# facebookresearch/multipathnet

Hardware: NVIDIA H100
Metric: proposals/sec (higher is better)
Workload: dtype fp32 (wgmma split emulation, fp32 accumulate: 3 bf16 products per MAC, 2 fp16 products in fc6/fc7)

## Files before the change

multipathnet_b200/csrc/gemm_tc.cu:

```cuda
#include "conv_gemm.cuh"
#include "wgmma.cuh"
#include "fp8_e4m3.cuh"
#include <algorithm>
#include <stdlib.h>
#include <string.h>

namespace {

constexpr int BM = 128;
constexpr int BK = 64;
constexpr int TC_THREADS = 384;
constexpr int CONS_THREADS = 256;
constexpr int A_TILE_BYTES = BM * BK * 2;
constexpr int SMEM_BUDGET = 196608;

__host__ __device__ constexpr int a_planes(OperandScheme ops) { return (ops == OperandScheme::BF16X1 || ops == OperandScheme::FP8X1) ? 1 : 2; }
__host__ __device__ constexpr int b_planes(OperandScheme ops) { return ops == OperandScheme::BF16X3 ? 2 : 1; }
__host__ __device__ constexpr int elem_bytes(OperandScheme ops) { return ops == OperandScheme::FP8X1 ? 1 : 2; }
__host__ __device__ constexpr int row_bytes(int BN, OperandScheme ops) { return (ops == OperandScheme::FP8X1 || BN == 256) ? 64 : 128; }
__host__ __device__ constexpr int stage_k(int BN, OperandScheme ops) { return row_bytes(BN, ops) / elem_bytes(ops); }
__host__ __device__ constexpr int kb_steps(int BN, OperandScheme ops) { return BK / stage_k(BN, ops); }
__host__ __device__ constexpr int a_tile_bytes(int BN, OperandScheme ops) { return BM * row_bytes(BN, ops); }
__host__ __device__ constexpr int stage_bytes(int BN, OperandScheme ops = OperandScheme::BF16X3) {
  return (a_planes(ops) * BM + b_planes(ops) * BN) * row_bytes(BN, ops);
}
__host__ __device__ constexpr int max_stages(int BN, OperandScheme ops) { return row_bytes(BN, ops) == 64 ? 8 : 4; }
__host__ __device__ constexpr int num_stages(int BN, OperandScheme ops = OperandScheme::BF16X3) {
  return (SMEM_BUDGET / stage_bytes(BN, ops)) > max_stages(BN, ops) ? max_stages(BN, ops) : (SMEM_BUDGET / stage_bytes(BN, ops));
}
__host__ __device__ constexpr int tc_smem_bytes(int BN, OperandScheme ops) {
  return num_stages(BN, ops) * stage_bytes(BN, ops) + 1024  + 256 ;
}
__host__ __device__ constexpr int stg_ld(int BN) { return BN + 4; }

struct TcParams {
  int N, Ho, Wo, Cout;
  int kh, kw, stride, pad;
  int cblocks;
  int tn, th, tw;
  int tiles_img, tiles_h, tiles_w, tiles_n;
  const float *bias;
  const __nv_bfloat16 *res_hi, *res_lo; long long res_ld;
  __nv_bfloat16 *out_hi, *out_lo; long long out_ld;
  float *out_f32; long long out_f32_ld;
  __nv_bfloat16 *pool_hi, *pool_lo; long long pool_ld; int Hp, Wp;
  int relu;
  int splitk, kb_per_split;
  long long split_stride;
  unsigned long long *tl_min, *tl_max;
  float acc_scale;
  int out_fmt;
  unsigned *ovf;
  const int *a_exp, *b_exp; long long sample_pix;
};

__device__ __forceinline__ unsigned long long gtimer() {
  unsigned long long t; asm volatile("mov.u64 %0, %%globaltimer;" : "=l"(t)); return t;
}
__device__ __forceinline__ void tl_min_stamp(const unsigned long long *base_, int i) {
  if (base_) atomicMin(const_cast<unsigned long long *>(base_) + i, gtimer());
}
__device__ __forceinline__ void tl_max_stamp(const unsigned long long *base_, int i) {
  if (base_) atomicMax(const_cast<unsigned long long *>(base_) + i, gtimer());
}
__device__ __forceinline__ uint32_t smem_u32(const void *p) { return (uint32_t)__cvta_generic_to_shared(p); }
__device__ __forceinline__ void mbar_init(uint32_t bar, uint32_t count) {
  asm volatile("mbarrier.init.shared::cta.b64 [%0], %1;" ::"r"(bar), "r"(count) : "memory");
}
__device__ __forceinline__ void mbar_expect_tx(uint32_t bar, uint32_t bytes) {
  asm volatile("mbarrier.arrive.expect_tx.shared::cta.b64 _, [%0], %1;" ::"r"(bar), "r"(bytes) : "memory");
}
__device__ __forceinline__ void mbar_arrive(uint32_t bar) {
  asm volatile("mbarrier.arrive.shared::cta.b64 _, [%0];" ::"r"(bar) : "memory");
}
__device__ __forceinline__ void mbar_wait(uint32_t bar, uint32_t parity) {
  uint32_t done;
  uint32_t spins = 0;
  do {
    asm volatile(
        "{\n\t.reg .pred p;\n\t"
        "mbarrier.try_wait.parity.shared::cta.b64 p, [%1], %2;\n\t"
        "selp.u32 %0, 1, 0, p;\n\t}"
        : "=r"(done) : "r"(bar), "r"(parity) : "memory");
    if (!done && ++spins == (1u << 26)) __trap();
  } while (!done);
}
__device__ __forceinline__ void tma_load_4d(uint32_t dst, const CUtensorMap *tm, uint32_t bar, int c0, int c1,
                                            int c2, int c3) {
  asm volatile(
      "cp.async.bulk.tensor.4d.shared::cluster.global.mbarrier::complete_tx::bytes [%0], [%1, {%3, %4, %5, %6}], [%2];"
      ::"r"(dst), "l"(reinterpret_cast<uint64_t>(tm)), "r"(bar), "r"(c0), "r"(c1), "r"(c2), "r"(c3) : "memory");
}
__device__ __forceinline__ void tma_load_2d(uint32_t dst, const CUtensorMap *tm, uint32_t bar, int c0, int c1) {
  asm volatile(
      "cp.async.bulk.tensor.2d.shared::cluster.global.mbarrier::complete_tx::bytes [%0], [%1, {%3, %4}], [%2];"
      ::"r"(dst), "l"(reinterpret_cast<uint64_t>(tm)), "r"(bar), "r"(c0), "r"(c1) : "memory");
}
__device__ __forceinline__ void prefetch_tmap(const CUtensorMap *tm) {
  asm volatile("prefetch.tensormap [%0];" ::"l"(reinterpret_cast<uint64_t>(tm)) : "memory");
}
__device__ __forceinline__ void consumers_sync() { asm volatile("bar.sync 1, 256;" ::: "memory"); }

__device__ __forceinline__ uint64_t make_smem_desc(uint32_t saddr) {
  uint64_t d = 0;
  d |= (uint64_t)((saddr & 0x3FFFFu) >> 4);
  d |= (uint64_t)1 << 16;
  d |= (uint64_t)(1024 >> 4) << 32;
  d |= (uint64_t)1 << 62;
  return d;
}

__device__ __forceinline__ uint64_t make_smem_desc_64b(uint32_t saddr) {
  uint64_t d = 0;
  d |= (uint64_t)((saddr & 0x3FFFFu) >> 4);
  d |= (uint64_t)1 << 16;
  d |= (uint64_t)(512 >> 4) << 32;
  d |= (uint64_t)2 << 62;
  return d;
}

template <int BN, OperandScheme OPS>
__device__ __forceinline__ void mma_kstep(float (&acc)[BN / 2], uint64_t a_hi, uint64_t a_lo, uint64_t b_hi, uint64_t b_lo, bool first) {
  constexpr bool F16 = (OPS == OperandScheme::FP16X2);
#pragma unroll
  for (int k = 0; k < stage_k(BN, OPS) / 16; ++k) {
    const uint64_t adv = (uint64_t)((k * 16 * 2) >> 4);
    const uint32_t later = (first && k == 0) ? 0u : 1u;
    if constexpr (OPS == OperandScheme::BF16X1) {
      wgmma_nk16<BN, false>(acc, a_hi + adv, b_hi + adv, later);
    } else {
      wgmma_nk16<BN, F16>(acc, a_lo + adv, b_hi + adv, later);
      if (!F16) wgmma_nk16<BN, F16>(acc, a_hi + adv, b_lo + adv, 1u);
      wgmma_nk16<BN, F16>(acc, a_hi + adv, b_hi + adv, 1u);
    }
  }
}

template <int BN>
__device__ __forceinline__ void stage_acc(float *stg, const float (&acc)[BN / 2], int g, int t) {
  const int r0 = g * 64 + (t >> 5) * 16 + ((t & 31) >> 2), c0 = 2 * (t & 3);
#pragma unroll
  for (int j = 0; j < BN / 8; ++j) {
    *reinterpret_cast<float2 *>(stg + r0 * stg_ld(BN) + 8 * j + c0) = make_float2(acc[4 * j], acc[4 * j + 1]);
    *reinterpret_cast<float2 *>(stg + (r0 + 8) * stg_ld(BN) + 8 * j + c0) = make_float2(acc[4 * j + 2], acc[4 * j + 3]);
  }
}

template <int BN, OperandScheme OPS>
__device__ __forceinline__ void epilogue_row(const TcParams &p, const float *srow, int nt, bool row_ok, long long pix,
                                             float *out_f32, int ch_first, long long ppix) {
  const bool pool = (p.pool_hi != nullptr);
  const int tile_end = min(p.Cout, nt * BN + BN);
#pragma unroll 1
  for (int ch = ch_first; ch < BN / 32; ch += 2) {
    const int col0 = nt * BN + ch * 32;
    if (col0 >= tile_end) break;
    float v[32];
#pragma unroll
    for (int j = 0; j < 8; ++j) {
      const float4 x = *reinterpret_cast<const float4 *>(srow + ch * 32 + 4 * j);
      v[4 * j] = x.x; v[4 * j + 1] = x.y; v[4 * j + 2] = x.z; v[4 * j + 3] = x.w;
    }
    if (OPS == OperandScheme::FP16X2) {
#pragma unroll
      for (int e = 0; e < 32; ++e) v[e] *= p.acc_scale;
    }
    if (OPS == OperandScheme::FP8X1) {
      const int ea = row_ok ? __ldg(p.a_exp + pix / p.sample_pix) : 0;
#pragma unroll
      for (int e = 0; e < 32; ++e) v[e] *= mpn_fp8::pow2(-(ea + __ldg(p.b_exp + col0 + e)));
    }
    if (!(row_ok || pool)) continue;
#pragma unroll
    for (int g = 0; g < 4; ++g) {
      const int c = col0 + g * 8;
      if (c >= tile_end) break;
      float f[8];
#pragma unroll
      for (int e = 0; e < 8; ++e) f[e] = v[g * 8 + e];
      const bool full8 = (c + 8 <= tile_end);
      if (p.bias) {
        if (full8) {
          const float4 b0 = __ldg(reinterpret_cast<const float4 *>(p.bias + c));
          const float4 b1 = __ldg(reinterpret_cast<const float4 *>(p.bias + c + 4));
          f[0] += b0.x; f[1] += b0.y; f[2] += b0.z; f[3] += b0.w;
          f[4] += b1.x; f[5] += b1.y; f[6] += b1.z; f[7] += b1.w;
        } else {
          for (int e = 0; e < 8 && c + e < p.Cout; ++e) f[e] += __ldg(p.bias + c + e);
        }
      }
      if (p.res_hi && full8 && row_ok) {
        const uint4 rh = *reinterpret_cast<const uint4 *>(p.res_hi + pix * p.res_ld + c);
        const uint4 rl = *reinterpret_cast<const uint4 *>(p.res_lo + pix * p.res_ld + c);
        const uint32_t hh[4] = {rh.x, rh.y, rh.z, rh.w}, ll[4] = {rl.x, rl.y, rl.z, rl.w};
#pragma unroll
        for (int t = 0; t < 4; ++t) {
          float2 x = bf16x2_to_float2(hh[t]), y = bf16x2_to_float2(ll[t]);
          f[2 * t] += x.x + y.x; f[2 * t + 1] += x.y + y.y;
        }
      }
      if (p.relu) {
#pragma unroll
        for (int e = 0; e < 8; ++e) f[e] = fmaxf(f[e], 0.f);
      }
      if (p.out_hi && full8 && row_ok) {
        uint32_t oh[4], ol[4];
#pragma unroll
        for (int t = 0; t < 4; ++t) split_x2(p.out_fmt, f[2 * t], f[2 * t + 1], oh[t], ol[t], p.ovf);
        *reinterpret_cast<uint4 *>(p.out_hi + pix * p.out_ld + c) = make_uint4(oh[0], oh[1], oh[2], oh[3]);
        *reinterpret_cast<uint4 *>(p.out_lo + pix * p.out_ld + c) = make_uint4(ol[0], ol[1], ol[2], ol[3]);
      }
      if (pool) {
#pragma unroll
        for (int e = 0; e < 8; ++e) {
          float x = row_ok ? f[e] : -INFINITY;
          x = fmaxf(x, __shfl_xor_sync(0xffffffffu, x, 1));
          x = fmaxf(x, __shfl_xor_sync(0xffffffffu, x, 8));
          f[e] = x;
        }
        if (ppix >= 0 && full8) {
          uint32_t oh[4], ol[4];
#pragma unroll
          for (int t = 0; t < 4; ++t) split_x2(p.out_fmt, f[2 * t], f[2 * t + 1], oh[t], ol[t], p.ovf);
          *reinterpret_cast<uint4 *>(p.pool_hi + ppix * p.pool_ld + c) = make_uint4(oh[0], oh[1], oh[2], oh[3]);
          *reinterpret_cast<uint4 *>(p.pool_lo + ppix * p.pool_ld + c) = make_uint4(ol[0], ol[1], ol[2], ol[3]);
        }
      }
      if (out_f32 && row_ok) {
        float *o = out_f32 + pix * p.out_f32_ld + c;
        if (full8 && ((reinterpret_cast<uintptr_t>(o) & 15) == 0)) {
          reinterpret_cast<float4 *>(o)[0] = make_float4(f[0], f[1], f[2], f[3]);
          reinterpret_cast<float4 *>(o)[1] = make_float4(f[4], f[5], f[6], f[7]);
        } else {
          for (int e = 0; e < 8 && c + e < p.Cout; ++e) o[e] = f[e];
        }
      }
    }
  }
}

template <int BN, OperandScheme OPS = OperandScheme::BF16X3>
__global__ void __launch_bounds__(TC_THREADS, 1)
conv_gemm_tc_kernel(const __grid_constant__ CUtensorMap tmA_hi, const __grid_constant__ CUtensorMap tmA_lo,
                    const __grid_constant__ CUtensorMap tmB_hi, const __grid_constant__ CUtensorMap tmB_lo,
                    const TcParams p) {
  constexpr int S = num_stages(BN, OPS);
  constexpr int STAGE = stage_bytes(BN, OPS);
  constexpr int A_TILE = a_tile_bytes(BN, OPS);
  constexpr int B_TILE_BYTES = BN * row_bytes(BN, OPS);
  constexpr int B_OFF = a_planes(OPS) * A_TILE;
  constexpr int KSTEPS = kb_steps(BN, OPS);
  static_assert(BM * stg_ld(BN) * 4 <= S * STAGE, "staging tile must fit in the ring");
  static_assert(S >= 2 && 2 * S * 8 <= 256, "ring depth: at least two stages, barriers in their 256 bytes");
  extern __shared__ uint8_t smem_raw[];
  uint8_t *smem = reinterpret_cast<uint8_t *>((reinterpret_cast<uintptr_t>(smem_raw) + 1023) & ~(uintptr_t)1023);
  uint64_t *bars = reinterpret_cast<uint64_t *>(smem + (size_t)S * STAGE);
  const uint32_t smem_base = smem_u32(smem);
  const uint32_t bar_base = smem_u32(bars);
  auto full_bar = [&](int s) { return bar_base + 8u * s; };
  auto empty_bar = [&](int s) { return bar_base + 8u * (S + s); };

  const int tid = threadIdx.x, lane = tid & 31;
  const int unit = (int)blockIdx.x;
  const int tile = unit / p.splitk, split = unit - tile * p.splitk;
  const int nt = tile % p.tiles_n, mt = tile / p.tiles_n;
  const int twi = mt % p.tiles_w, thi = (mt / p.tiles_w) % p.tiles_h, tni = mt / (p.tiles_w * p.tiles_h);
  const int num_kb = p.kh * p.kw * p.cblocks;
  const int kb0 = split * p.kb_per_split, kb1 = min(num_kb, kb0 + p.kb_per_split);

  if (tid == 0) {
    tl_min_stamp(p.tl_min, 0);
    if (a_planes(OPS) == 1) { prefetch_tmap(&tmA_hi); prefetch_tmap(&tmB_hi); }
    else { prefetch_tmap(&tmA_hi); prefetch_tmap(&tmA_lo); prefetch_tmap(&tmB_hi); prefetch_tmap(&tmB_lo); }
    for (int s = 0; s < S; ++s) { mbar_init(full_bar(s), 1); mbar_init(empty_bar(s), CONS_THREADS / 32); }
    asm volatile("fence.mbarrier_init.release.cluster;" ::: "memory");
  }
  __syncthreads();
  asm volatile("griddepcontrol.wait;" ::: "memory");
  asm volatile("griddepcontrol.launch_dependents;" ::: "memory");
  if (tid == 0) tl_min_stamp(p.tl_min, 1);

  if (tid < 128) {
    if (tid == 0) {
      const int w_in0 = twi * p.tw * p.stride - p.pad, h_in0 = thi * p.th * p.stride - p.pad, n0 = tni * p.tn;
      const int b_row0 = nt * BN;
      for (int kb = kb0, it = 0; kb < kb1; ++kb) {
        const int tap = kb / p.cblocks, cb = kb - tap * p.cblocks;
        const int khi = tap / p.kw, kwi = tap - khi * p.kw;
#pragma unroll
        for (int h = 0; h < KSTEPS; ++h, ++it) {
          const int s = it % S; const uint32_t ph = (uint32_t)(it / S) & 1u;
          const int ka = cb * BK + h * stage_k(BN, OPS), kk = kb * BK + h * stage_k(BN, OPS);
          mbar_wait(empty_bar(s), ph ^ 1u);
          const uint32_t sa = smem_base + (uint32_t)s * STAGE;
          mbar_expect_tx(full_bar(s), (uint32_t)STAGE);
          tma_load_4d(sa, &tmA_hi, full_bar(s), ka, w_in0 + kwi, h_in0 + khi, n0);
          if (a_planes(OPS) == 2) tma_load_4d(sa + A_TILE, &tmA_lo, full_bar(s), ka, w_in0 + kwi, h_in0 + khi, n0);
          tma_load_2d(sa + B_OFF, &tmB_hi, full_bar(s), kk, b_row0);
          if (b_planes(OPS) == 2) tma_load_2d(sa + B_OFF + B_TILE_BYTES, &tmB_lo, full_bar(s), kk, b_row0);
        }
      }
    }
    return;
  }

  const int e = tid - 128;
  const int g = e >> 7, t = e & 127;
  float acc[BN / 2];
#pragma unroll
  for (int i = 0; i < BN / 2; ++i) acc[i] = 0.f;
  if constexpr (OPS == OperandScheme::FP8X1) {
    float part[BN / 2];
#pragma unroll
    for (int i = 0; i < BN / 2; ++i) part[i] = 0.f;
    for (int kb = kb0, it = 0; kb < kb1; ++kb, ++it) {
      const int s = it % S; const uint32_t ph = (uint32_t)(it / S) & 1u;
      mbar_wait(full_bar(s), ph);
      if (it == 0 && e == 0) tl_min_stamp(p.tl_min, 2);
      const uint32_t sa = smem_base + (uint32_t)s * STAGE;
      const uint64_t a8 = make_smem_desc_64b(sa + (uint32_t)g * (A_TILE / 2));
      const uint64_t b8 = make_smem_desc_64b(sa + B_OFF);
#pragma unroll
      for (int k = 0; k < BK / 32; ++k) {
        wgmma_fence_acc(part);
        wgmma_fence();
        wgmma_e4m3_nk32<BN>(part, a8 + (uint64_t)(2 * k), b8 + (uint64_t)(2 * k), 0u);
        wgmma_commit();
        wgmma_wait<0>();
        wgmma_fence_acc(part);
#pragma unroll
        for (int i = 0; i < BN / 2; ++i) acc[i] += part[i];
      }
      if (lane == 0) mbar_arrive(empty_bar(s));
    }
  } else {
  const int steps = (kb1 - kb0) * KSTEPS;
  for (int it = 0; it < steps; ++it) {
    const int s = it % S; const uint32_t ph = (uint32_t)(it / S) & 1u;
    mbar_wait(full_bar(s), ph);
    if (it == 0 && e == 0) tl_min_stamp(p.tl_min, 2);
    const uint32_t sa = smem_base + (uint32_t)s * STAGE;
    auto desc = [](uint32_t a) { return row_bytes(BN, OPS) == 64 ? make_smem_desc_64b(a) : make_smem_desc(a); };
    const uint64_t a_hi = desc(sa + (uint32_t)g * (A_TILE / 2));
    const uint64_t a_lo = desc(sa + A_TILE + (uint32_t)g * (A_TILE / 2));
    const uint64_t b_hi = desc(sa + B_OFF);
    const uint64_t b_lo = desc(sa + B_OFF + B_TILE_BYTES);
    wgmma_fence_acc(acc);
    wgmma_fence();
    mma_kstep<BN, OPS>(acc, a_hi, a_lo, b_hi, b_lo, it == 0);
    wgmma_commit();
    wgmma_wait<1>();
    wgmma_fence_acc(acc);
    if (it > 0 && lane == 0) mbar_arrive(empty_bar((it - 1) % S));
  }
  wgmma_wait<0>();
  wgmma_fence_acc(acc);
  }
  if (e == 0) tl_max_stamp(p.tl_max, 0);
  consumers_sync();
  float *stg = reinterpret_cast<float *>(smem);
  stage_acc<BN>(stg, acc, g, t);
  consumers_sync();

  const int row = e & 127;
  const int wl = row & (p.tw - 1), hl = (row / p.tw) & (p.th - 1), nl = row / (p.tw * p.th);
  const int wo = twi * p.tw + wl, ho = thi * p.th + hl, n = tni * p.tn + nl;
  const bool row_ok = (wo < p.Wo) && (ho < p.Ho) && (n < p.N);
  const long long pix = ((long long)n * p.Ho + ho) * p.Wo + wo;
  const long long ppix = (p.pool_hi && row_ok && !(lane & 9)) ? ((long long)n * p.Hp + (ho >> 1)) * p.Wp + (wo >> 1) : -1;
  float *const out_f32 = p.out_f32 ? p.out_f32 + (long long)split * p.split_stride : nullptr;
  epilogue_row<BN, OPS>(p, stg + row * stg_ld(BN), nt, row_ok, pix, out_f32, e >> 7, ppix);
  if (e == 0) tl_max_stamp(p.tl_max, 1);
}

constexpr int C1_THREADS = 256;
constexpr int C1_A_BYTES = 2 * A_TILE_BYTES;
constexpr int C1_B_BYTES = 2 * 64 * 128;
constexpr int C1_OUT_WARP = 16 * 128;
constexpr int C1_SMEM = 2 * C1_A_BYTES + C1_B_BYTES + (C1_THREADS / 32) * C1_OUT_WARP + 1024;

__device__ __forceinline__ void conv1_gather(const float *__restrict__ x, int pix, int pixels, int H, int W, int bhalf,
                                             float (&in)[16]) {
#pragma unroll
  for (int k = 0; k < 16; ++k) in[k] = 0.f;
  if (pix < pixels) {
    const int HW = H * W;
    const int n = pix / HW, rem = pix - n * HW;
    const int ho = rem / W, wo = rem - ho * W;
    const float *x0 = x + ((size_t)n * 3 * HW + (size_t)(ho - 1) * W + (wo - 1));
    const bool rok[3] = {ho >= 1, true, ho + 1 < H}, cok[3] = {wo >= 1, true, wo + 1 < W};
#pragma unroll
    for (int k = 0; k < 16; ++k) {
      const int kk = 16 * bhalf + k;
      if (kk < 27) {
        const int ci = kk / 9, r = (kk / 3) % 3, q = kk % 3;
        in[k] = (rok[r] && cok[q]) ? __ldg(x0 + ci * HW + r * W + q) : 0.f;
      }
    }
  }
}

__device__ __forceinline__ void conv1_store_plane(uint32_t so, const uint32_t (&v)[16], __nv_bfloat16 *out, int pix0,
                                                  int pixels, int lane) {
  const int r = lane >> 2;
  const uint32_t wr = so + (uint32_t)(r * 128 + 4 * (lane & 3));
  __syncwarp();
#pragma unroll
  for (int j = 0; j < 8; ++j) {
    const uint32_t a = wr + (uint32_t)((j ^ r) * 16);
    asm volatile("st.shared.b32 [%0], %1;" ::"r"(a), "r"(v[j]) : "memory");
    asm volatile("st.shared.b32 [%0], %1;" ::"r"(a + 8 * 128), "r"(v[8 + j]) : "memory");
  }
  __syncwarp();
  const int row0 = lane >> 3, ch = lane & 7;
  const uint32_t rd0 = so + (uint32_t)(row0 * 128 + ((ch ^ row0) * 16)), rd1 = so + (uint32_t)(row0 * 128 + ((ch ^ row0 ^ 4) * 16));
  __nv_bfloat16 *o = out + (size_t)(pix0 + row0) * 64 + ch * 8;
#pragma unroll
  for (int q = 0; q < 4; ++q) {
    uint4 d;
    asm volatile("ld.shared.v4.b32 {%0, %1, %2, %3}, [%4];" : "=r"(d.x), "=r"(d.y), "=r"(d.z), "=r"(d.w)
                 : "r"(((q & 1) ? rd1 : rd0) + (uint32_t)(q * 4 * 128)) : "memory");
    if (pix0 + row0 + 4 * q < pixels) *reinterpret_cast<uint4 *>(o + q * 4 * 64) = d;
  }
}

__global__ void __launch_bounds__(C1_THREADS, 2)
conv1_tc_kernel(const float *__restrict__ x, int N, int H, int W, const float *__restrict__ w, const float *__restrict__ bias,
                int relu, __nv_bfloat16 *__restrict__ out_hi, __nv_bfloat16 *__restrict__ out_lo) {
  extern __shared__ uint8_t smem_raw[];
  uint8_t *smem = reinterpret_cast<uint8_t *>((reinterpret_cast<uintptr_t>(smem_raw) + 1023) & ~(uintptr_t)1023);
  uint8_t *sB = smem + 2 * C1_A_BYTES;
  const int tid = threadIdx.x, lane = tid & 31, warp = tid >> 5;
  const uint32_t so = smem_u32(sB + C1_B_BYTES) + (uint32_t)(warp * C1_OUT_WARP);
  const uint32_t b_base = smem_u32(sB);
  const int g = tid >> 7;
  const int pixels = N * H * W;
  const int total_tiles = (pixels + BM - 1) / BM;
  asm volatile("griddepcontrol.wait;" ::: "memory");
  asm volatile("griddepcontrol.launch_dependents;" ::: "memory");
  const int c0 = 2 * (lane & 3);
  for (int i = tid; i < 64 * 4; i += C1_THREADS) {
    const int row = i >> 2, j = i & 3;
    uint32_t hh[4], ll[4];
#pragma unroll
    for (int q = 0; q < 4; ++q) {
      const int k0 = j * 8 + 2 * q;
      const float v0 = (k0 < 27) ? __ldg(w + row * 27 + k0) : 0.f, v1 = (k0 + 1 < 27) ? __ldg(w + row * 27 + k0 + 1) : 0.f;
      split_bf16x2(v0, v1, hh[q], ll[q]);
    }
    const uint32_t off = (uint32_t)row * 128u + (uint32_t)((j ^ (row & 7)) * 16);
    *reinterpret_cast<uint4 *>(sB + off) = make_uint4(hh[0], hh[1], hh[2], hh[3]);
    *reinterpret_cast<uint4 *>(sB + 64 * 128 + off) = make_uint4(ll[0], ll[1], ll[2], ll[3]);
  }
  const int brow = tid & 127, bhalf = tid >> 7;
  float in[16];
  conv1_gather(x, (int)blockIdx.x * BM + brow, pixels, H, W, bhalf, in);
// ... 52 lines not shown
#pragma unroll
        for (int h = 0; h < 2; ++h) {
          uint32_t hi2, lo2;
          split_bf16x2(acc[4 * j + 2 * h], acc[4 * j + 2 * h + 1], hi2, lo2);
          v[8 * h + j] = plane ? lo2 : hi2;
        }
      conv1_store_plane(so, v, plane ? out_lo : out_hi, pix0, pixels, lane);
    }
  }
}

struct ReduceParams {
  const float *ws; long long split_stride; int splitk; long long pixels; int Cout;
  const float *bias; const __nv_bfloat16 *res_hi, *res_lo; long long res_ld; int relu;
  __nv_bfloat16 *out_hi, *out_lo; long long out_ld; float *out_f32; long long out_f32_ld;
  OutScatter scatter;
};
__global__ void __launch_bounds__(256) splitk_reduce_kernel(const ReduceParams r) {
  MPN_PDL_SYNC();
  const long long idx = (long long)blockIdx.x * blockDim.x + threadIdx.x;
  if (idx >= r.pixels * r.Cout) return;
  const long long pix = idx / r.Cout; const int c = (int)(idx - pix * r.Cout);
  float acc = 0.f;
  for (int s = 0; s < r.splitk; ++s) acc += r.ws[(long long)s * r.split_stride + idx];
  if (r.bias) acc += __ldg(r.bias + c);
  if (r.res_hi) acc += join_bf16(r.res_hi[pix * r.res_ld + c], r.res_lo[pix * r.res_ld + c]);
  if (r.relu) acc = fmaxf(acc, 0.f);
  if (r.out_hi) { __nv_bfloat16 h, l; split_bf16(acc, h, l); r.out_hi[pix * r.out_ld + c] = h; r.out_lo[pix * r.out_ld + c] = l; }
  if (r.scatter.n > 0) {
#pragma unroll 1
    for (int g = 0; g < r.scatter.n; ++g)
      if (c >= r.scatter.seg[g].c0 && c < r.scatter.seg[g].c1) { r.scatter.seg[g].ptr[pix * r.scatter.seg[g].ld + (c - r.scatter.seg[g].c0)] = acc; break; }
  } else if (r.out_f32) r.out_f32[pix * r.out_f32_ld + c] = acc;
}

typedef CUresult (*PFN_encodeTiled)(CUtensorMap *, CUtensorMapDataType, cuuint32_t, void *, const cuuint64_t *,
                                    const cuuint64_t *, const cuuint32_t *, const cuuint32_t *, CUtensorMapInterleave,
                                    CUtensorMapSwizzle, CUtensorMapL2promotion, CUtensorMapFloatOOBfill);
PFN_encodeTiled get_encode_fn() {
  static PFN_encodeTiled fn = nullptr;
  if (!fn) {
    void *p = nullptr; cudaDriverEntryPointQueryResult q;
    if (cudaGetDriverEntryPoint("cuTensorMapEncodeTiled", &p, cudaEnableDefault, &q) == cudaSuccess &&
        q == cudaDriverEntryPointSuccess)
      fn = reinterpret_cast<PFN_encodeTiled>(p);
  }
  return fn;
}

int encode_map(mpn_ctx *ctx, CUtensorMap *tm, const void *base, int rank, const cuuint64_t *dims,
               const cuuint64_t *strides_bytes , const cuuint32_t *box, const cuuint32_t *estr, int BN, OperandScheme ops) {
  const bool fp8 = ops == OperandScheme::FP8X1;
  PFN_encodeTiled fn = get_encode_fn();
  if (!fn) return mpn_fail(ctx, MPN_ERR_CUDA, "cuTensorMapEncodeTiled entry point unavailable");
  CUresult r = fn(tm, fp8 ? CU_TENSOR_MAP_DATA_TYPE_UINT8 : CU_TENSOR_MAP_DATA_TYPE_BFLOAT16, (cuuint32_t)rank, const_cast<void *>(base), dims,
                  strides_bytes, box, estr, CU_TENSOR_MAP_INTERLEAVE_NONE, row_bytes(BN, ops) == 64 ? CU_TENSOR_MAP_SWIZZLE_64B : CU_TENSOR_MAP_SWIZZLE_128B,
                  CU_TENSOR_MAP_L2_PROMOTION_L2_256B, CU_TENSOR_MAP_FLOAT_OOB_FILL_NONE);
  if (r != CUDA_SUCCESS) {
    char b[256];
    snprintf(b, sizeof b, "cuTensorMapEncodeTiled failed (%d): rank %d dims %llu %llu box %u %u", (int)r, rank,
             (unsigned long long)dims[0], (unsigned long long)dims[1], box[0], box[1]);
    return mpn_fail(ctx, MPN_ERR_CUDA, b);
  }
  return MPN_OK;
}

inline bool tc_use_pdl() {
  static const int on = [] { const char *e = getenv("MPN_TC_PDL"); return (e && e[0] == '0') ? 0 : 1; }();
  return on != 0;
}

template <int BN, OperandScheme OPS = OperandScheme::BF16X3>
int launch_bn(mpn_ctx *ctx, const ConvPlan &pl, const TcParams &tp) {
  const int smem = tc_smem_bytes(BN, OPS);
  constexpr int bslot = BN == 256 ? 2 : (BN == 128 ? 1 : 0);
  constexpr int slot = OPS == OperandScheme::FP16X2 ? 3 : (OPS == OperandScheme::BF16X1 ? 5 + bslot
                                                         : (OPS == OperandScheme::FP8X1 ? 8 + bslot : bslot));
  if (!ctx->tc_attr_set[slot]) {
    MPN_CUDA(ctx, cudaFuncSetAttribute(conv_gemm_tc_kernel<BN, OPS>, cudaFuncAttributeMaxDynamicSharedMemorySize, smem));
    ctx->tc_attr_set[slot] = 1;
  }
  const long long units = (long long)pl.tiles_img * pl.tiles_h * pl.tiles_w * pl.tiles_n * pl.splitk;
  MPN_CHECK_ARG(ctx, units > 0 && units < (1ll << 31), "conv_tc: grid size out of range");
  cudaLaunchConfig_t cfg = {};
  cfg.gridDim = dim3((unsigned)units); cfg.blockDim = dim3(TC_THREADS); cfg.dynamicSmemBytes = (size_t)smem; cfg.stream = ctx->stream;
  cudaLaunchAttribute attr[1];
  int na = 0;
  if (tc_use_pdl()) {
    attr[na].id = cudaLaunchAttributeProgrammaticStreamSerialization;
    attr[na].val.programmaticStreamSerializationAllowed = 1;
    ++na;
  }
  cfg.attrs = attr; cfg.numAttrs = na;
  MPN_CUDA(ctx, cudaLaunchKernelEx(&cfg, conv_gemm_tc_kernel<BN, OPS>, pl.tmA_hi, pl.tmA_lo, pl.tmB_hi, pl.tmB_lo, tp));
  MPN_LAUNCHED(ctx);
  return MPN_OK;
}

int launch_ops(mpn_ctx *ctx, const ConvPlan &pl, const TcParams &tp) {
  if (pl.ops == OperandScheme::FP16X2) return launch_bn<256, OperandScheme::FP16X2>(ctx, pl, tp);
  if (pl.ops == OperandScheme::FP8X1)
    return pl.BN == 128 ? launch_bn<128, OperandScheme::FP8X1>(ctx, pl, tp) : launch_bn<64, OperandScheme::FP8X1>(ctx, pl, tp);
  if (pl.ops == OperandScheme::BF16X1) {
    switch (pl.BN) {
      case 256: return launch_bn<256, OperandScheme::BF16X1>(ctx, pl, tp);
      case 128: return launch_bn<128, OperandScheme::BF16X1>(ctx, pl, tp);
      default: return launch_bn<64, OperandScheme::BF16X1>(ctx, pl, tp);
    }
  }
  switch (pl.BN) {
    case 256: return launch_bn<256>(ctx, pl, tp);
    case 128: return launch_bn<128>(ctx, pl, tp);
    default: return launch_bn<64>(ctx, pl, tp);
  }
}

}

int conv1_tc_launch(mpn_ctx *ctx, const float *x_nchw, int N, int H, int W, const float *w_dev, const float *bias_dev, int relu,
                    DTensor &y) {
  MPN_CHECK_ARG(ctx, y.hi && y.lo && y.C == 64 && y.ld % 8 == 0, "conv1_tc: output must be 64-channel split planes");
  MPN_CHECK_ARG(ctx, bias_dev, "conv1_tc: bias missing");
  MPN_CHECK_ARG(ctx, y.ld == 64 && (long long)N * H * W < (1ll << 31) - 256, "conv1_tc: dense 64-channel output and < 2^31 pixels");
  if (!ctx->tc_attr_set[4]) {
    MPN_CUDA(ctx, cudaFuncSetAttribute(conv1_tc_kernel, cudaFuncAttributeMaxDynamicSharedMemorySize, C1_SMEM));
    ctx->tc_attr_set[4] = 1;
  }
  const long long tiles = ((long long)N * H * W + BM - 1) / BM;
  cudaLaunchConfig_t cfg = {};
  cfg.gridDim = dim3((unsigned)std::min<long long>(tiles, 2ll * ctx->sm_count)); cfg.blockDim = dim3(C1_THREADS);
  cfg.dynamicSmemBytes = (size_t)C1_SMEM; cfg.stream = ctx->stream;
  cudaLaunchAttribute attr[1];
  int na = 0;
  if (tc_use_pdl()) { attr[na].id = cudaLaunchAttributeProgrammaticStreamSerialization; attr[na].val.programmaticStreamSerializationAllowed = 1; ++na; }
  cfg.attrs = attr; cfg.numAttrs = na;
  MPN_CUDA(ctx, cudaLaunchKernelEx(&cfg, conv1_tc_kernel, x_nchw, N, H, W, w_dev, bias_dev, relu, y.hi, y.lo));
  MPN_LAUNCHED(ctx);
  return MPN_OK;
}

double conv_flops(const ConvProblem &p) {
  const double Ho = (double)p.y.H, Wo = (double)p.y.W;
  return 2.0 * (double)p.x.C * p.Cout * p.kh * p.kw * Ho * Wo * (double)p.y.N;
}

static int conv_tc_plan_impl(mpn_ctx *ctx, int sm_count, const ConvProblem &p, ConvPlan &pl, bool choose_only) {
  pl.valid = 0;
  MPN_CHECK_ARG(ctx, choose_only || (p.x.hi && p.x.lo && ((p.w_hi && p.w_lo) || p.w16)), "conv_tc: operands must be split-bf16 (or an fp16 weight plane)");
  MPN_CHECK_ARG(ctx, !(p.w16 && p.bf16), "conv_tc: the bf16 numerics do not take an fp16 weight plane");
  MPN_CHECK_ARG(ctx, !(p.fp8 && (p.w16 || p.bf16)), "conv_tc: the fp8 numerics take neither an fp16 weight plane nor the bf16 numerics");
  MPN_CHECK_ARG(ctx, choose_only || !p.fp8 || (p.x8 && p.x8_exp && p.w8 && p.w8_exp), "conv_tc: the fp8 numerics need e4m3 planes and exponents");
  pl.ops = p.w16 ? OperandScheme::FP16X2 : (p.fp8 ? OperandScheme::FP8X1 : (p.bf16 ? OperandScheme::BF16X1 : OperandScheme::BF16X3));
  const bool w16 = pl.ops == OperandScheme::FP16X2, fp8 = pl.ops == OperandScheme::FP8X1;
  MPN_CHECK_ARG(ctx, choose_only || (p.x.fmt == 1) == w16, "conv_tc: fp16 activation planes go with the fp16 weight plane (and only with it)");
  MPN_CHECK_ARG(ctx, p.x.C % BK == 0, "conv_tc: Cin must be a multiple of 64");
  MPN_CHECK_ARG(ctx, p.x.ld % 8 == 0, "conv_tc: input pixel stride must be a multiple of 8 elements");
  MPN_CHECK_ARG(ctx, p.stride >= 1 && p.stride <= 2, "conv_tc: stride must be 1 or 2");
  const int Ho = (int)p.y.H, Wo = (int)p.y.W, N = (int)p.y.N;
  pl.flat = (p.kh == 1 && p.kw == 1 && p.stride == 1 && p.pad == 0) ? 1 : 0;
  pl.mode = 0; pl.splitk = 1;
  cuuint64_t dims[4], strides[3]; cuuint32_t box[4], estr[4];
  int gtn = 1, gth = 1, gtw = BM;
  if (!pl.flat) {
    double best = -1.0;
    for (int tw = 1; tw <= 128; tw <<= 1)
      for (int th = 1; th * tw <= 128; th <<= 1) {
        const int tn = 128 / (tw * th);
        if (tw * p.stride > 256 || th * p.stride > 256) continue;
        const long long tiles = (long long)((Wo + tw - 1) / tw) * ((Ho + th - 1) / th) * ((N + tn - 1) / tn);
        const double util = (double)N * Ho * Wo / (double)(tiles * 128) + 1e-6 * tw;
        if (util > best) { best = util; gtn = tn; gth = th; gtw = tw; }
      }
  }
  const long long P = (long long)p.x.N * p.x.H * p.x.W;
  {
    const bool r3_ok = (p.kh == 3 && p.kw == 3 && p.stride == 1 && p.pad == 1);
    const char *env3 = getenv("MPN_TC_R3");
// ... 160 lines not shown
```

Measured before the change: 320,100.

## Make conv GEMM kernel persistent with register-direct epilogue and register reallocation

Launches at most one CTA per SM and loops over tiles, so the TMA producer can prefetch the next tile's stages while consumers run the current tile's epilogue. The epilogue no longer stages the whole fp32 accumulator tile through the ring buffer. Each warp now writes bf16 hi/lo pieces straight from registers through a small swizzled per-warp shared buffer for coalesced stores, with pooling done by warp shuffles. setmaxnreg moves registers from the producer warpgroup to the consumers. The risks are reduced parallelism when there are fewer units than SMs, more epilogue complexity, and changed bounds handling in the residual and fp32 paths.

```diff
diff --git a/multipathnet_b200/csrc/gemm_tc.cu b/multipathnet_b200/csrc/gemm_tc.cu
--- a/multipathnet_b200/csrc/gemm_tc.cu
+++ b/multipathnet_b200/csrc/gemm_tc.cu
@@ -28,10 +28,11 @@
 __host__ __device__ constexpr int num_stages(int BN, OperandScheme ops = OperandScheme::BF16X3) {
   return (SMEM_BUDGET / stage_bytes(BN, ops)) > max_stages(BN, ops) ? max_stages(BN, ops) : (SMEM_BUDGET / stage_bytes(BN, ops));
 }
+constexpr int EPI_WARP_BYTES = 16 * 128;
+constexpr int EPI_BYTES = (CONS_THREADS / 32) * EPI_WARP_BYTES;
 __host__ __device__ constexpr int tc_smem_bytes(int BN, OperandScheme ops) {
-  return num_stages(BN, ops) * stage_bytes(BN, ops) + 1024  + 256 ;
-}
-__host__ __device__ constexpr int stg_ld(int BN) { return BN + 4; }
+  return num_stages(BN, ops) * stage_bytes(BN, ops) + EPI_BYTES + 1024  + 256 ;
+}
 
 struct TcParams {
   int N, Ho, Wo, Cout;
@@ -39,6 +40,7 @@
   int cblocks;
   int tn, th, tw;
   int tiles_img, tiles_h, tiles_w, tiles_n;
+  int units;
   const float *bias;
   const __nv_bfloat16 *res_hi, *res_lo; long long res_ld;
   __nv_bfloat16 *out_hi, *out_lo; long long out_ld;
@@ -99,7 +101,6 @@
 __device__ __forceinline__ void prefetch_tmap(const CUtensorMap *tm) {
   asm volatile("prefetch.tensormap [%0];" ::"l"(reinterpret_cast<uint64_t>(tm)) : "memory");
 }
-__device__ __forceinline__ void consumers_sync() { asm volatile("bar.sync 1, 256;" ::: "memory"); }
 
 __device__ __forceinline__ uint64_t make_smem_desc(uint32_t saddr) {
   uint64_t d = 0;
@@ -136,106 +137,161 @@
   }
 }
 
-template <int BN>
-__device__ __forceinline__ void stage_acc(float *stg, const float (&acc)[BN / 2], int g, int t) {
-  const int r0 = g * 64 + (t >> 5) * 16 + ((t & 31) >> 2), c0 = 2 * (t & 3);
-#pragma unroll
-  for (int j = 0; j < BN / 8; ++j) {
-    *reinterpret_cast<float2 *>(stg + r0 * stg_ld(BN) + 8 * j + c0) = make_float2(acc[4 * j], acc[4 * j + 1]);
-    *reinterpret_cast<float2 *>(stg + (r0 + 8) * stg_ld(BN) + 8 * j + c0) = make_float2(acc[4 * j + 2], acc[4 * j + 3]);
+struct UnitPos { int nt, twi, thi, tni, split; };
+__device__ __forceinline__ UnitPos unit_pos(const TcParams &p, int unit) {
+  UnitPos u;
+  const int tile = unit / p.splitk;
+  u.split = unit - tile * p.splitk;
+  u.nt = tile % p.tiles_n;
+  const int mt = tile / p.tiles_n;
+  u.twi = mt % p.tiles_w; u.thi = (mt / p.tiles_w) % p.tiles_h; u.tni = mt / (p.tiles_w * p.tiles_h);
+  return u;
+}
+__device__ __forceinline__ long long row_pixel(const TcParams &p, const UnitPos &u, int row, bool &ok, int *whn = nullptr) {
+  const int lw = __ffs(p.tw) - 1, lh = __ffs(p.th) - 1;
+  const int wl = row & (p.tw - 1), hl = (row >> lw) & (p.th - 1), nl = row >> (lw + lh);
+  const int wo = u.twi * p.tw + wl, ho = u.thi * p.th + hl, n = u.tni * p.tn + nl;
+  ok = (wo < p.Wo) && (ho < p.Ho) && (n < p.N);
+  if (whn) { whn[0] = wo; whn[1] = ho; whn[2] = n; }
+  return ((long long)n * p.Ho + ho) * p.Wo + wo;
+}
+
+__device__ __forceinline__ void store_plane_chunk(uint32_t so, const uint32_t (&v)[16], __nv_bfloat16 *out, long long ld,
+                                                  const TcParams &p, const UnitPos &u, int rbase, int col0, int lane) {
+  const int r = lane >> 2;
+  const uint32_t wr = so + (uint32_t)(r * 128 + 4 * (lane & 3));
+  __syncwarp();
+#pragma unroll
+  for (int j = 0; j < 8; ++j) {
+    const uint32_t a = wr + (uint32_t)((j ^ r) * 16);
+    asm volatile("st.shared.b32 [%0], %1;" ::"r"(a), "r"(v[j]) : "memory");
+    asm volatile("st.shared.b32 [%0], %1;" ::"r"(a + 8 * 128), "r"(v[8 + j]) : "memory");
+  }
+  __syncwarp();
+  const int row0 = lane >> 3, ch = lane & 7;
+  const uint32_t rd0 = so + (uint32_t)(row0 * 128 + ((ch ^ row0) * 16)), rd1 = so + (uint32_t)(row0 * 128 + ((ch ^ row0 ^ 4) * 16));
+  const bool col_ok = col0 + 8 * ch < p.Cout;
+#pragma unroll
+  for (int q = 0; q < 4; ++q) {
+    uint4 d;
+    asm volatile("ld.shared.v4.b32 {%0, %1, %2, %3}, [%4];" : "=r"(d.x), "=r"(d.y), "=r"(d.z), "=r"(d.w)
+                 : "r"(((q & 1) ? rd1 : rd0) + (uint32_t)(q * 4 * 128)) : "memory");
+    bool ok;
+    const long long pix = row_pixel(p, u, rbase + 4 * q + row0, ok);
+    if (ok && col_ok) *reinterpret_cast<uint4 *>(out + pix * ld + col0 + 8 * ch) = d;
   }
 }
 
 template <int BN, OperandScheme OPS>
-__device__ __forceinline__ void epilogue_row(const TcParams &p, const float *srow, int nt, bool row_ok, long long pix,
-                                             float *out_f32, int ch_first, long long ppix) {
+__device__ __forceinline__ void tile_epilogue(const TcParams &p, const UnitPos &u, float (&acc)[BN / 2], int g, int wq,
+                                              int lane, uint32_t so) {
+  const int rbase = 64 * g + 16 * wq;
+  const int c0 = 2 * (lane & 3);
+  bool fok[2]; long long fpix[2];
+#pragma unroll
+  for (int i = 0; i < 2; ++i) fpix[i] = row_pixel(p, u, rbase + (lane >> 2) + 8 * i, fok[i]);
+  int ea[2] = {0, 0};
+  if constexpr (OPS == OperandScheme::FP8X1) {
+#pragma unroll
+    for (int i = 0; i < 2; ++i) ea[i] = fok[i] ? __ldg(p.a_exp + fpix[i] / p.sample_pix) : 0;
+  }
   const bool pool = (p.pool_hi != nullptr);
-  const int tile_end = min(p.Cout, nt * BN + BN);
+  bool pok = false; long long ppix = 0;
+  if (pool) {
+    int whn[3];
+    row_pixel(p, u, rbase + 2 * (lane >> 3), pok, whn);
+    ppix = ((long long)whn[2] * p.Hp + (whn[1] >> 1)) * p.Wp + (whn[0] >> 1);
+  }
+  float *const out_f32 = p.out_f32 ? p.out_f32 + (long long)u.split * p.split_stride : nullptr;
 #pragma unroll 1
-  for (int ch = ch_first; ch < BN / 32; ch += 2) {
-    const int col0 = nt * BN + ch * 32;
-    if (col0 >= tile_end) break;
-    float v[32];
+  for (int m = 0; m < BN / 64; ++m) {
+    const int col0 = u.nt * BN + 64 * m;
+    if (col0 >= p.Cout) break;
+    float *f = acc;
 #pragma unroll
     for (int j = 0; j < 8; ++j) {
-      const float4 x = *reinterpret_cast<const float4 *>(srow + ch * 32 + 4 * j);
-      v[4 * j] = x.x; v[4 * j + 1] = x.y; v[4 * j + 2] = x.z; v[4 * j + 3] = x.w;
-    }
-    if (OPS == OperandScheme::FP16X2) {
-#pragma unroll
-      for (int e = 0; e < 32; ++e) v[e] *= p.acc_scale;
-    }
-    if (OPS == OperandScheme::FP8X1) {
-      const int ea = row_ok ? __ldg(p.a_exp + pix / p.sample_pix) : 0;
-#pragma unroll
-      for (int e = 0; e < 32; ++e) v[e] *= mpn_fp8::pow2(-(ea + __ldg(p.b_exp + col0 + e)));
-    }
-    if (!(row_ok || pool)) continue;
-#pragma unroll
-    for (int g = 0; g < 4; ++g) {
-      const int c = col0 + g * 8;
-      if (c >= tile_end) break;
-      float f[8];
-#pragma unroll
-      for (int e = 0; e < 8; ++e) f[e] = v[g * 8 + e];
-      const bool full8 = (c + 8 <= tile_end);
-      if (p.bias) {
-        if (full8) {
-          const float4 b0 = __ldg(reinterpret_cast<const float4 *>(p.bias + c));
-          const float4 b1 = __ldg(reinterpret_cast<const float4 *>(p.bias + c + 4));
-          f[0] += b0.x; f[1] += b0.y; f[2] += b0.z; f[3] += b0.w;
-          f[4] += b1.x; f[5] += b1.y; f[6] += b1.z; f[7] += b1.w;
-        } else {
-          for (int e = 0; e < 8 && c + e < p.Cout; ++e) f[e] += __ldg(p.bias + c + e);
+      const int c = col0 + 8 * j + c0;
+      const bool full8 = col0 + 8 * j + 8 <= p.Cout;
+      float b[2] = {0.f, 0.f};
+      int eb[2] = {0, 0};
+#pragma unroll
+      for (int k = 0; k < 2; ++k) {
+        if (p.bias && c + k < p.Cout) b[k] = __ldg(p.bias + c + k);
+        if constexpr (OPS == OperandScheme::FP8X1) eb[k] = __ldg(p.b_exp + c + k);
+      }
+#pragma unroll
+      for (int i = 0; i < 2; ++i) {
+        float &f0 = f[4 * j + 2 * i], &f1 = f[4 * j + 2 * i + 1];
+        if constexpr (OPS == OperandScheme::FP16X2) { f0 *= p.acc_scale; f1 *= p.acc_scale; }
+        if constexpr (OPS == OperandScheme::FP8X1) {
+          f0 *= mpn_fp8::pow2(-(ea[i] + eb[0])); f1 *= mpn_fp8::pow2(-(ea[i] + eb[1]));
+        }
+        if (p.bias) {
+          if (c < p.Cout) f0 += b[0];
+          if (c + 1 < p.Cout) f1 += b[1];
+        }
+        if (p.res_hi && full8 && fok[i]) {
+          const float2 x = bf16x2_to_float2(*reinterpret_cast<const uint32_t *>(p.res_hi + fpix[i] * p.res_ld + c));
+          const float2 y = bf16x2_to_float2(*reinterpret_cast<const uint32_t *>(p.res_lo + fpix[i] * p.res_ld + c));
+          f0 += x.x + y.x; f1 += x.y + y.y;
+        }
+        if (p.relu) { f0 = fmaxf(f0, 0.f); f1 = fmaxf(f1, 0.f); }
+        if (out_f32 && fok[i]) {
+          float *o = out_f32 + fpix[i] * p.out_f32_ld + c;
+          if (c < p.Cout) o[0] = f0;
+          if (c + 1 < p.Cout) o[1] = f1;
         }
       }
-      if (p.res_hi && full8 && row_ok) {
-        const uint4 rh = *reinterpret_cast<const uint4 *>(p.res_hi + pix * p.res_ld + c);
-        const uint4 rl = *reinterpret_cast<const uint4 *>(p.res_lo + pix * p.res_ld + c);
-        const uint32_t hh[4] = {rh.x, rh.y, rh.z, rh.w}, ll[4] = {rl.x, rl.y, rl.z, rl.w};
-#pragma unroll
-        for (int t = 0; t < 4; ++t) {
-          float2 x = bf16x2_to_float2(hh[t]), y = bf16x2_to_float2(ll[t]);
-          f[2 * t] += x.x + y.x; f[2 * t + 1] += x.y + y.y;
+    }
+    float mx[16];
+    if (pool) {
+#pragma unroll
+      for (int j = 0; j < 8; ++j)
+#pragma unroll
+        for (int k = 0; k < 2; ++k) {
+          float top = fok[0] ? f[4 * j + k] : -INFINITY, bot = fok[1] ? f[4 * j + 2 + k] : -INFINITY;
+          top = fmaxf(top, __shfl_xor_sync(0xffffffffu, top, 4));
+          bot = fmaxf(bot, __shfl_xor_sync(0xffffffffu, bot, 4));
+          mx[2 * j + k] = fmaxf(top, bot);
         }
-      }
-      if (p.relu) {
-#pragma unroll
-        for (int e = 0; e < 8; ++e) f[e] = fmaxf(f[e], 0.f);
-      }
-      if (p.out_hi && full8 && row_ok) {
-        uint32_t oh[4], ol[4];
-#pragma unroll
-        for (int t = 0; t < 4; ++t) split_x2(p.out_fmt, f[2 * t], f[2 * t + 1], oh[t], ol[t], p.ovf);
-        *reinterpret_cast<uint4 *>(p.out_hi + pix * p.out_ld + c) = make_uint4(oh[0], oh[1], oh[2], oh[3]);
-        *reinterpret_cast<uint4 *>(p.out_lo + pix * p.out_ld + c) = make_uint4(ol[0], ol[1], ol[2], ol[3]);
+    }
+#pragma unroll 1
+    for (int plane = 0; plane < 2; ++plane) {
+      if (p.out_hi) {
+        uint32_t v[16];
+#pragma unroll
+        for (int j = 0; j < 8; ++j)
+#pragma unroll
+          for (int i = 0; i < 2; ++i) {
+            uint32_t hi2 = 0, lo2 = 0;
+            if (fok[i]) split_x2(p.out_fmt, f[4 * j + 2 * i], f[4 * j + 2 * i + 1], hi2, lo2, p.ovf);
+            v[8 * i + j] = plane ? lo2 : hi2;
+          }
+        store_plane_chunk(so, v, plane ? p.out_lo : p.out_hi, p.out_ld, p, u, rbase, col0, lane);
       }
       if (pool) {
-#pragma unroll
-        for (int e = 0; e < 8; ++e) {
-          float x = row_ok ? f[e] : -INFINITY;
-          x = fmaxf(x, __shfl_xor_sync(0xffffffffu, x, 1));
-          x = fmaxf(x, __shfl_xor_sync(0xffffffffu, x, 8));
-          f[e] = x;
+        const int pr = lane >> 3;
+        __syncwarp();
+        if (!(lane & 4) && fok[0]) {
+#pragma unroll
+          for (int j = 0; j < 8; ++j) {
+            uint32_t hi2, lo2;
+            split_x2(p.out_fmt, mx[2 * j], mx[2 * j + 1], hi2, lo2, p.ovf);
+            const uint32_t a = so + (uint32_t)(pr * 128 + ((j ^ pr) * 16) + 4 * (lane & 3));
+            asm volatile("st.shared.b32 [%0], %1;" ::"r"(a), "r"(plane ? lo2 : hi2) : "memory");
+          }
         }
-        if (ppix >= 0 && full8) {
-          uint32_t oh[4], ol[4];
-#pragma unroll
-          for (int t = 0; t < 4; ++t) split_x2(p.out_fmt, f[2 * t], f[2 * t + 1], oh[t], ol[t], p.ovf);
-          *reinterpret_cast<uint4 *>(p.pool_hi + ppix * p.pool_ld + c) = make_uint4(oh[0], oh[1], oh[2], oh[3]);
-          *reinterpret_cast<uint4 *>(p.pool_lo + ppix * p.pool_ld + c) = make_uint4(ol[0], ol[1], ol[2], ol[3]);
-        }
+        __syncwarp();
+        const int ch = lane & 7;
+        uint4 d;
+        asm volatile("ld.shared.v4.b32 {%0, %1, %2, %3}, [%4];" : "=r"(d.x), "=r"(d.y), "=r"(d.z), "=r"(d.w)
+                     : "r"(so + (uint32_t)(pr * 128 + ((ch ^ pr) * 16))) : "memory");
+        if (pok && col0 + 8 * ch < p.Cout)
+          *reinterpret_cast<uint4 *>((plane ? p.pool_lo : p.pool_hi) + ppix * p.pool_ld + col0 + 8 * ch) = d;
       }
-      if (out_f32 && row_ok) {
-        float *o = out_f32 + pix * p.out_f32_ld + c;
-        if (full8 && ((reinterpret_cast<uintptr_t>(o) & 15) == 0)) {
-          reinterpret_cast<float4 *>(o)[0] = make_float4(f[0], f[1], f[2], f[3]);
-          reinterpret_cast<float4 *>(o)[1] = make_float4(f[4], f[5], f[6], f[7]);
-        } else {
-          for (int e = 0; e < 8 && c + e < p.Cout; ++e) o[e] = f[e];
-        }
-      }
-    }
+    }
+#pragma unroll
+    for (int k = 0; k + 32 < BN / 2; ++k) acc[k] = acc[k + 32];
   }
 }
 
@@ -250,23 +306,17 @@
   constexpr int B_TILE_BYTES = BN * row_bytes(BN, OPS);
   constexpr int B_OFF = a_planes(OPS) * A_TILE;
   constexpr int KSTEPS = kb_steps(BN, OPS);
-  static_assert(BM * stg_ld(BN) * 4 <= S * STAGE, "staging tile must fit in the ring");
   static_assert(S >= 2 && 2 * S * 8 <= 256, "ring depth: at least two stages, barriers in their 256 bytes");
   extern __shared__ uint8_t smem_raw[];
   uint8_t *smem = reinterpret_cast<uint8_t *>((reinterpret_cast<uintptr_t>(smem_raw) + 1023) & ~(uintptr_t)1023);
-  uint64_t *bars = reinterpret_cast<uint64_t *>(smem + (size_t)S * STAGE);
+  uint64_t *bars = reinterpret_cast<uint64_t *>(smem + (size_t)S * STAGE + EPI_BYTES);
   const uint32_t smem_base = smem_u32(smem);
   const uint32_t bar_base = smem_u32(bars);
   auto full_bar = [&](int s) { return bar_base + 8u * s; };
   auto empty_bar = [&](int s) { return bar_base + 8u * (S + s); };
 
   const int tid = threadIdx.x, lane = tid & 31;
-  const int unit = (int)blockIdx.x;
-  const int tile = unit / p.splitk, split = unit - tile * p.splitk;
-  const int nt = tile % p.tiles_n, mt = tile / p.tiles_n;
-  const int twi = mt % p.tiles_w, thi = (mt / p.tiles_w) % p.tiles_h, tni = mt / (p.tiles_w * p.tiles_h);
   const int num_kb = p.kh * p.kw * p.cblocks;
-  const int kb0 = split * p.kb_per_split, kb1 = min(num_kb, kb0 + p.kb_per_split);
 
   if (tid == 0) {
     tl_min_stamp(p.tl_min, 0);
@@ -281,97 +331,104 @@
   if (tid == 0) tl_min_stamp(p.tl_min, 1);
 
   if (tid < 128) {
+    asm volatile("setmaxnreg.dec.sync.aligned.u32 24;" ::: "memory");
     if (tid == 0) {
-      const int w_in0 = twi * p.tw * p.stride - p.pad, h_in0 = thi * p.th * p.stride - p.pad, n0 = tni * p.tn;
-      const int b_row0 = nt * BN;
-      for (int kb = kb0, it = 0; kb < kb1; ++kb) {
-        const int tap = kb / p.cblocks, cb = kb - tap * p.cblocks;
-        const int khi = tap / p.kw, kwi = tap - khi * p.kw;
-#pragma unroll
-        for (int h = 0; h < KSTEPS; ++h, ++it) {
-          const int s = it % S; const uint32_t ph = (uint32_t)(it / S) & 1u;
-          const int ka = cb * BK + h * stage_k(BN, OPS), kk = kb * BK + h * stage_k(BN, OPS);
-          mbar_wait(empty_bar(s), ph ^ 1u);
-          const uint32_t sa = smem_base + (uint32_t)s * STAGE;
-          mbar_expect_tx(full_bar(s), (uint32_t)STAGE);
-          tma_load_4d(sa, &tmA_hi, full_bar(s), ka, w_in0 + kwi, h_in0 + khi, n0);
-          if (a_planes(OPS) == 2) tma_load_4d(sa + A_TILE, &tmA_lo, full_bar(s), ka, w_in0 + kwi, h_in0 + khi, n0);
-          tma_load_2d(sa + B_OFF, &tmB_hi, full_bar(s), kk, b_row0);
-          if (b_planes(OPS) == 2) tma_load_2d(sa + B_OFF + B_TILE_BYTES, &tmB_lo, full_bar(s), kk, b_row0);
+      int it = 0;
+      for (int unit = (int)blockIdx.x; unit < p.units; unit += (int)gridDim.x) {
+        const UnitPos u = unit_pos(p, unit);
+        const int kb0 = u.split * p.kb_per_split, kb1 = min(num_kb, kb0 + p.kb_per_split);
+        const int w_in0 = u.twi * p.tw * p.stride - p.pad, h_in0 = u.thi * p.th * p.stride - p.pad, n0 = u.tni * p.tn;
+        const int b_row0 = u.nt * BN;
+        for (int kb = kb0; kb < kb1; ++kb) {
+          const int tap = kb / p.cblocks, cb = kb - tap * p.cblocks;
+          const int khi = tap / p.kw, kwi = tap - khi * p.kw;
+#pragma unroll
+          for (int h = 0; h < KSTEPS; ++h, ++it) {
+            const int s = it % S; const uint32_t ph = (uint32_t)(it / S) & 1u;
+            const int ka = cb * BK + h * stage_k(BN, OPS), kk = kb * BK + h * stage_k(BN, OPS);
+            mbar_wait(empty_bar(s), ph ^ 1u);
+            const uint32_t sa = smem_base + (uint32_t)s * STAGE;
+            mbar_expect_tx(full_bar(s), (uint32_t)STAGE);
+            tma_load_4d(sa, &tmA_hi, full_bar(s), ka, w_in0 + kwi, h_in0 + khi, n0);
+            if (a_planes(OPS) == 2) tma_load_4d(sa + A_TILE, &tmA_lo, full_bar(s), ka, w_in0 + kwi, h_in0 + khi, n0);
+            tma_load_2d(sa + B_OFF, &tmB_hi, full_bar(s), kk, b_row0);
+            if (b_planes(OPS) == 2) tma_load_2d(sa + B_OFF + B_TILE_BYTES, &tmB_lo, full_bar(s), kk, b_row0);
+          }
         }
       }
     }
     return;
   }
 
+  asm volatile("setmaxnreg.inc.sync.aligned.u32 240;" ::: "memory");
   const int e = tid - 128;
-  const int g = e >> 7, t = e & 127;
-  float acc[BN / 2];
-#pragma unroll
-  for (int i = 0; i < BN / 2; ++i) acc[i] = 0.f;
-  if constexpr (OPS == OperandScheme::FP8X1) {
-    float part[BN / 2];
-#pragma unroll
-    for (int i = 0; i < BN / 2; ++i) part[i] = 0.f;
-    for (int kb = kb0, it = 0; kb < kb1; ++kb, ++it) {
-      const int s = it % S; const uint32_t ph = (uint32_t)(it / S) & 1u;
-      mbar_wait(full_bar(s), ph);
-      if (it == 0 && e == 0) tl_min_stamp(p.tl_min, 2);
-      const uint32_t sa = smem_base + (uint32_t)s * STAGE;
-      const uint64_t a8 = make_smem_desc_64b(sa + (uint32_t)g * (A_TILE / 2));
-      const uint64_t b8 = make_smem_desc_64b(sa + B_OFF);
-#pragma unroll
-      for (int k = 0; k < BK / 32; ++k) {
-        wgmma_fence_acc(part);
+  const int g = e >> 7, wq = (e >> 5) & 3;
+  const uint32_t so = smem_base + (uint32_t)(S * STAGE + (e >> 5) * EPI_WARP_BYTES);
+  int it = 0;
+  for (int unit = (int)blockIdx.x; unit < p.units; unit += (int)gridDim.x) {
+    const UnitPos u = unit_pos(p, unit);
+    const int kb0 = u.split * p.kb_per_split, kb1 = min(num_kb, kb0 + p.kb_per_split);
+    float acc[BN / 2];
+#pragma unroll
+    for (int i = 0; i < BN / 2; ++i) acc[i] = 0.f;
+    if constexpr (OPS == OperandScheme::FP8X1) {
+      float part[BN / 2];
+#pragma unroll
+      for (int i = 0; i < BN / 2; ++i) part[i] = 0.f;
+      for (int kb = kb0; kb < kb1; ++kb, ++it) {
+        const int s = it % S; const uint32_t ph = (uint32_t)(it / S) & 1u;
+        mbar_wait(full_bar(s), ph);
+        if (it == 0 && e == 0) tl_min_stamp(p.tl_min, 2);
+        const uint32_t sa = smem_base + (uint32_t)s * STAGE;
+        const uint64_t a8 = make_smem_desc_64b(sa + (uint32_t)g * (A_TILE / 2));
+        const uint64_t b8 = make_smem_desc_64b(sa + B_OFF);
+#pragma unroll
+        for (int k = 0; k < BK / 32; ++k) {
+          wgmma_fence_acc(part);
+          wgmma_fence();
+          wgmma_e4m3_nk32<BN>(part, a8 + (uint64_t)(2 * k), b8 + (uint64_t)(2 * k), 0u);
+          wgmma_commit();
+          wgmma_wait<0>();
+          wgmma_fence_acc(part);
+#pragma unroll
+          for (int i = 0; i < BN / 2; ++i) acc[i] += part[i];
+        }
+        if (lane == 0) mbar_arrive(empty_bar(s));
+      }
+    } else {
+      const int steps = (kb1 - kb0) * KSTEPS;
+      for (int i = 0; i < steps; ++i, ++it) {
+        const int s = it % S; const uint32_t ph = (uint32_t)(it / S) & 1u;
+        mbar_wait(full_bar(s), ph);
+        if (it == 0 && e == 0) tl_min_stamp(p.tl_min, 2);
+        const uint32_t sa = smem_base + (uint32_t)s * STAGE;
+        auto desc = [](uint32_t a) { return row_bytes(BN, OPS) == 64 ? make_smem_desc_64b(a) : make_smem_desc(a); };
+        const uint64_t a_hi = desc(sa + (uint32_t)g * (A_TILE / 2));
+        const uint64_t a_lo = desc(sa + A_TILE + (uint32_t)g * (A_TILE / 2));
+        const uint64_t b_hi = desc(sa + B_OFF);
+        const uint64_t b_lo = desc(sa + B_OFF + B_TILE_BYTES);
+        wgmma_fence_acc(acc);
         wgmma_fence();
-        wgmma_e4m3_nk32<BN>(part, a8 + (uint64_t)(2 * k), b8 + (uint64_t)(2 * k), 0u);
+        mma_kstep<BN, OPS>(acc, a_hi, a_lo, b_hi, b_lo, i == 0);
         wgmma_commit();
-        wgmma_wait<0>();
-        wgmma_fence_acc(part);
-#pragma unroll
-        for (int i = 0; i < BN / 2; ++i) acc[i] += part[i];
+        wgmma_wait<1>();
+        wgmma_fence_acc(acc);
+        if (i > 0 && lane == 0) mbar_arrive(empty_bar((it - 1) % S));
       }
-      if (lane == 0) mbar_arrive(empty_bar(s));
-    }
-  } else {
-  const int steps = (kb1 - kb0) * KSTEPS;
-  for (int it = 0; it < steps; ++it) {
-    const int s = it % S; const uint32_t ph = (uint32_t)(it / S) & 1u;
-    mbar_wait(full_bar(s), ph);
-    if (it == 0 && e == 0) tl_min_stamp(p.tl_min, 2);
-    const uint32_t sa = smem_base + (uint32_t)s * STAGE;
-    auto desc = [](uint32_t a) { return row_bytes(BN, OPS) == 64 ? make_smem_desc_64b(a) : make_smem_desc(a); };
-    const uint64_t a_hi = desc(sa + (uint32_t)g * (A_TILE / 2));
-    const uint64_t a_lo = desc(sa + A_TILE + (uint32_t)g * (A_TILE / 2));
-    const uint64_t b_hi = desc(sa + B_OFF);
-    const uint64_t b_lo = desc(sa + B_OFF + B_TILE_BYTES);
-    wgmma_fence_acc(acc);
-    wgmma_fence();
-    mma_kstep<BN, OPS>(acc, a_hi, a_lo, b_hi, b_lo, it == 0);
-    wgmma_commit();
-    wgmma_wait<1>();
-    wgmma_fence_acc(acc);
-    if (it > 0 && lane == 0) mbar_arrive(empty_bar((it - 1) % S));
-  }
-  wgmma_wait<0>();
-  wgmma_fence_acc(acc);
-  }
-  if (e == 0) tl_max_stamp(p.tl_max, 0);
-  consumers_sync();
-  float *stg = reinterpret_cast<float *>(smem);
-  stage_acc<BN>(stg, acc, g, t);
-  consumers_sync();
-
-  const int row = e & 127;
-  const int wl = row & (p.tw - 1), hl = (row / p.tw) & (p.th - 1), nl = row / (p.tw * p.th);
-  const int wo = twi * p.tw + wl, ho = thi * p.th + hl, n = tni * p.tn + nl;
-  const bool row_ok = (wo < p.Wo) && (ho < p.Ho) && (n < p.N);
-  const long long pix = ((long long)n * p.Ho + ho) * p.Wo + wo;
-  const long long ppix = (p.pool_hi && row_ok && !(lane & 9)) ? ((long long)n * p.Hp + (ho >> 1)) * p.Wp + (wo >> 1) : -1;
-  float *const out_f32 = p.out_f32 ? p.out_f32 + (long long)split * p.split_stride : nullptr;
-  epilogue_row<BN, OPS>(p, stg + row * stg_ld(BN), nt, row_ok, pix, out_f32, e >> 7, ppix);
-  if (e == 0) tl_max_stamp(p.tl_max, 1);
-}
+      wgmma_wait<0>();
+      wgmma_fence_acc(acc);
+      if (lane == 0) mbar_arrive(empty_bar((it - 1) % S));
+    }
+    if (e == 0) tl_max_stamp(p.tl_max, 0);
+    const uint32_t t_epi = (p.tl_max && e == 0) ? (uint32_t)gtimer() : 0u;
+    tile_epilogue<BN, OPS>(p, u, acc, g, wq, lane, so);
+    if (e == 0) {
+      tl_max_stamp(p.tl_max, 1);
+      if (p.tl_max) atomicAdd(p.tl_max + 3, (unsigned long long)((uint32_t)gtimer() - t_epi));
+    }
+  }
+}
+
 
 constexpr int C1_THREADS = 256;
 constexpr int C1_A_BYTES = 2 * A_TILE_BYTES;
@@ -590,8 +647,11 @@
   }
   const long long units = (long long)pl.tiles_img * pl.tiles_h * pl.tiles_w * pl.tiles_n * pl.splitk;
   MPN_CHECK_ARG(ctx, units > 0 && units < (1ll << 31), "conv_tc: grid size out of range");
+  TcParams tpu = tp;
+  tpu.units = (int)units;
   cudaLaunchConfig_t cfg = {};
-  cfg.gridDim = dim3((unsigned)units); cfg.blockDim = dim3(TC_THREADS); cfg.dynamicSmemBytes = (size_t)smem; cfg.stream = ctx->stream;
+  cfg.gridDim = dim3((unsigned)std::min<long long>(units, ctx->sm_count));
+  cfg.blockDim = dim3(TC_THREADS); cfg.dynamicSmemBytes = (size_t)smem; cfg.stream = ctx->stream;
   cudaLaunchAttribute attr[1];
   int na = 0;
   if (tc_use_pdl()) {
@@ -600,7 +660,7 @@
     ++na;
   }
   cfg.attrs = attr; cfg.numAttrs = na;
-  MPN_CUDA(ctx, cudaLaunchKernelEx(&cfg, conv_gemm_tc_kernel<BN, OPS>, pl.tmA_hi, pl.tmA_lo, pl.tmB_hi, pl.tmB_lo, tp));
+  MPN_CUDA(ctx, cudaLaunchKernelEx(&cfg, conv_gemm_tc_kernel<BN, OPS>, pl.tmA_hi, pl.tmA_lo, pl.tmB_hi, pl.tmB_lo, tpu));
   MPN_LAUNCHED(ctx);
   return MPN_OK;
 }
```

New measurement: 334,700, median of 6. 1.05x the previous value.
